# aleflabo/PREGO

Measured on AMD Instinct MI355X. Metric: frames/sec (per-frame action logits) on Assembly101-O TSN features, higher is better.
Workload: dtype fp16; 1 GPU; BASELINE configs[1]: Assembly101-O-test-split-shaped eval set, MiniROAD eval path (rgb+flow fp32 [T,2048] each -> per-frame probs[86] + argmax); clips_per_gpu=182, frames_per_gpu=2306143, min_T=3342, max_T=33981, flow=non-zero (full K=4096 layer1 GEMM), parallelism=clip-sharded dp1, no collective: every rank its own eval-set-sized clip list, weights=random init, seed 20

## Files before the change

### prego_amd/csrc/head_softmax.hip

```cpp
#include "common.h"
#include "kernels.h"
#include <cstdlib>

#define HM 4
template <typename WT, int NTC>
__global__ __launch_bounds__(256) void head_softmax_kernel(
    const WT* __restrict__ Hrelu,
    const WT* __restrict__ Wc,
    const float* __restrict__ bc,
    SlotPlan plan, int row0, int nrows, int HID, int C, int apply_softmax,
    float* const* __restrict__ out_ptrs,
    int* const* __restrict__ argmax_ptrs) {
  constexpr bool BF = (sizeof(WT) == 2);
  const int lane = threadIdx.x & 63, wave = threadIdx.x >> 6;
  const int l15 = lane & 15, l4 = lane >> 4;
  const int rbase = (blockIdx.x * 4 + wave) * 16 * HM;
  if (rbase >= nrows) return;
  int arow[HM];
#pragma unroll
  for (int m = 0; m < HM; ++m) { arow[m] = rbase + m * 16 + l15; if (arow[m] > nrows - 1) arow[m] = nrows - 1; }

  __shared__ unsigned long long s_out[4][64], s_arg[4][64];
  {
    typedef const __attribute__((address_space(4))) int* cint_p;
    cint_p ro_c = (cint_p)plan.rowoff;
    int lo = 0, hi = plan.s_max;
    const int first = __builtin_amdgcn_readfirstlane(row0 + rbase);
    while (hi - lo > 1) {
      const int mid = (lo + hi) >> 1;
      if (ro_c[mid] <= first) lo = mid; else hi = mid;
    }
    int myrow = rbase + lane; if (myrow > nrows - 1) myrow = nrows - 1;
    myrow += row0;
    int a = lo, b = lo + 64 < plan.s_max ? lo + 64 : plan.s_max;
    if (plan.rowoff[b] <= myrow) { a = b; b = plan.s_max; }
    while (b - a > 1) {
      const int mid = (a + b) >> 1;
      if (plan.rowoff[mid] <= myrow) a = mid; else b = mid;
    }
    const int slot = myrow - plan.rowoff[a];
    int k = plan.seg_off[slot];
    const int kend = plan.seg_off[slot + 1];
    while (k + 1 < kend && plan.seg_start[k + 1] <= a) ++k;
    const int clip = plan.seg_clip[k], t = a - plan.seg_start[k];
    float* op = out_ptrs ? out_ptrs[clip] : nullptr;
    int* ap = argmax_ptrs ? argmax_ptrs[clip] : nullptr;
    s_out[wave][lane] = op ? (unsigned long long)(op + (size_t)t * C) : 0ull;
    s_arg[wave][lane] = ap ? (unsigned long long)(ap + t) : 0ull;
  }

  f32x4 acc[HM][NTC];
#pragma unroll
  for (int m = 0; m < HM; ++m)
#pragma unroll
    for (int j = 0; j < NTC; ++j) acc[m][j] = (f32x4){0.f, 0.f, 0.f, 0.f};

  if constexpr (BF) {
    const bf16_t* bp = (const bf16_t*)Wc + (size_t)l15 * HID + 8 * l4;
    for (int k = 0; k < HID; k += 32) {
      bf16x8 af[HM];
#pragma unroll
      for (int m = 0; m < HM; ++m) af[m] = *(const bf16x8*)((const bf16_t*)Hrelu + (size_t)arow[m] * HID + 8 * l4 + k);
#pragma unroll
      for (int j = 0; j < NTC; ++j) {
        const bf16x8 bfr = *(const bf16x8*)(bp + (size_t)j * 16 * HID + k);
#pragma unroll
        for (int m = 0; m < HM; ++m) acc[m][j] = op16<WT>::mfma(af[m], bfr, acc[m][j]);
      }
    }
  } else {
    const float* bp = (const float*)Wc + (size_t)l15 * HID + 4 * l4;
    for (int k = 0; k < HID; k += 16) {
      float4 af[HM];
#pragma unroll
      for (int m = 0; m < HM; ++m) af[m] = *(const float4*)((const float*)Hrelu + (size_t)arow[m] * HID + 4 * l4 + k);
#pragma unroll
      for (int j = 0; j < NTC; ++j) {
        const float4 bv = *(const float4*)(bp + (size_t)j * 16 * HID + k);
#pragma unroll
        for (int m = 0; m < HM; ++m) {
          acc[m][j] = __builtin_amdgcn_mfma_f32_16x16x4f32(af[m].x, bv.x, acc[m][j], 0, 0, 0);
          acc[m][j] = __builtin_amdgcn_mfma_f32_16x16x4f32(af[m].y, bv.y, acc[m][j], 0, 0, 0);
          acc[m][j] = __builtin_amdgcn_mfma_f32_16x16x4f32(af[m].z, bv.z, acc[m][j], 0, 0, 0);
          acc[m][j] = __builtin_amdgcn_mfma_f32_16x16x4f32(af[m].w, bv.w, acc[m][j], 0, 0, 0);
        }
      }
    }
  }

#pragma unroll
  for (int m = 0; m < HM; ++m)
#pragma unroll
  for (int e = 0; e < 4; ++e) {
    float v[NTC];
    float mx = -INFINITY;
    int mi = 0x7fffffff;
#pragma unroll
    for (int j = 0; j < NTC; ++j) {
      const int c = j * 16 + l15;
      v[j] = acc[m][j][e] + bc[c];
      if (c < C && v[j] > mx) { mx = v[j]; mi = c; }
    }
#pragma unroll
    for (int o = 1; o < 16; o <<= 1) {
      const float omx = __shfl_xor(mx, o, 64);
      const int omi = __shfl_xor(mi, o, 64);
      if (omx > mx || (omx == mx && omi < mi)) { mx = omx; mi = omi; }
    }
    float s = 0.f;
    if (apply_softmax) {
#pragma unroll
      for (int j = 0; j < NTC; ++j) {
        const int c = j * 16 + l15;
        v[j] = (c < C) ? __expf(v[j] - mx) : 0.f;
        s += v[j];
      }
#pragma unroll
      for (int o = 1; o < 16; o <<= 1) s += __shfl_xor(s, o, 64);
      const float inv = 1.0f / s;
#pragma unroll
      for (int j = 0; j < NTC; ++j) v[j] *= inv;
    }
    const int rr = m * 16 + l4 * 4 + e;
    if (rbase + rr < nrows) {
      float* op = (float*)s_out[wave][rr];
      if (op) {
#pragma unroll
        for (int j = 0; j < NTC; ++j) {
          const int c = j * 16 + l15;
          if (c < C) op[c] = v[j];
        }
      }
      if (l15 == 0) {
        int* aptr = (int*)s_arg[wave][rr];
        if (aptr) *aptr = mi;
      }
    }
  }
}

template <int NTC, typename OT = bf16_t>
__global__ __launch_bounds__(256, 1) void head_softmax_v2_kernel(
    const bf16_t* __restrict__ Hrelu, const bf16_t* __restrict__ Wc, const float* __restrict__ bc, SlotPlan plan, int row0,
    int nrows, int C, int apply_softmax, float* const* __restrict__ out_ptrs, int* const* __restrict__ argmax_ptrs,
    const int2* __restrict__ rowmap ) {
  constexpr int HID = 1024, KS = 8;
  extern __shared__ __attribute__((aligned(16))) char smem[];
  f32x4* part = (f32x4*)smem;
  constexpr int PSTRIDE = 4 * 2 * NTC * 64;
  const int lane = threadIdx.x & 63, q = __builtin_amdgcn_readfirstlane(threadIdx.x >> 6);
  const int l15 = lane & 15, g = lane >> 4;
  bf16x8 wc[NTC][KS];
#pragma unroll
  for (int j = 0; j < NTC; ++j)
#pragma unroll
    for (int ks = 0; ks < KS; ++ks) wc[j][ks] = *(const bf16x8*)(Wc + (size_t)(j * 16 + l15) * HID + q * 256 + ks * 32 + 8 * g);
  float bias[NTC][4];
#pragma unroll
  for (int j = 0; j < NTC; ++j)
#pragma unroll
    for (int e = 0; e < 4; ++e) bias[j][e] = bc[j * 16 + 4 * g + e];

  const int nblk = (nrows + 31) / 32;
  const int* __restrict__ p_rowoff = plan.rowoff; const int* __restrict__ p_seg_off = plan.seg_off;
  const int* __restrict__ p_seg_clip = plan.seg_clip; const int* __restrict__ p_seg_start = plan.seg_start;
  const int* __restrict__ p_blk = plan.blk_step;
  const int s_max = plan.s_max;
  bf16x8 cur[2][KS], nxt[2][KS];
#define HEAD_LOAD(DST, BLK)                                                                                             \
  do {                                                                                                                  \
    _Pragma("unroll") for (int t = 0; t < 2; ++t) {                                                                     \
      int r_ = (BLK) * 32 + t * 16 + l15; if (r_ > nrows - 1) r_ = nrows - 1;                                           \
      _Pragma("unroll") for (int ks = 0; ks < KS; ++ks) {                                                               \
        const u32x4 v_ = __builtin_nontemporal_load((const u32x4*)(Hrelu + (size_t)r_ * HID + q * 256 + ks * 32 + 8 * g)); \
        DST[t][ks] = __builtin_bit_cast(bf16x8, v_);                                                                    \
      }                                                                                                                 \
    }                                                                                                                   \
  } while (0)
  const int rq = (q & 1) * 16 + l15;
  auto map_row = [&](int b) { int r = b * 32 + rq; return r < nrows ? r : nrows - 1; };
  int blk = blockIdx.x;
  int2 ct = make_int2(0, 0), ctn = make_int2(0, 0);
  if (blk < nblk) {
    if (rowmap != nullptr) ct = rowmap[map_row(blk)];
    HEAD_LOAD(cur, blk);
  }
  int parity = 0;
  for (; blk < nblk; blk += gridDim.x) {
    const int bn = blk + gridDim.x;
    const int bnc = bn < nblk ? bn : blk;
    float* op_raw = nullptr; int* ap_raw = nullptr;
    if (rowmap != nullptr) {
      op_raw = out_ptrs ? out_ptrs[ct.x] : nullptr;
      ap_raw = argmax_ptrs ? argmax_ptrs[ct.x] : nullptr;
      ctn = rowmap[map_row(bnc)];
    }
    __builtin_amdgcn_sched_barrier(0);
    HEAD_LOAD(nxt, bnc);
    __builtin_amdgcn_sched_barrier(0);
    float* op = nullptr; int* ap = nullptr;
    const int myrow = blk * 32 + q * 16 + l15;
    if (q < 2 && myrow < nrows && rowmap == nullptr) {
      const int row = row0 + myrow;
      int lo = p_blk[row >> 5];
      while (lo + 1 < s_max && p_rowoff[lo + 1] <= row) ++lo;
      const int slot = row - p_rowoff[lo];
      int k = p_seg_off[slot];
      const int kend = p_seg_off[slot + 1];
      while (k + 1 < kend && p_seg_start[k + 1] <= lo) ++k;
      const int clip = p_seg_clip[k], t = lo - p_seg_start[k];
      op = out_ptrs ? out_ptrs[clip] : nullptr;
      if (op) op += (size_t)t * C;
      ap = argmax_ptrs ? argmax_ptrs[clip] : nullptr;
      if (ap) ap += t;
    }
    f32x4 acc[2][NTC];
#pragma unroll
    for (int t = 0; t < 2; ++t)
#pragma unroll
      for (int j = 0; j < NTC; ++j) acc[t][j] = (f32x4){0.f, 0.f, 0.f, 0.f};
#pragma unroll
    for (int ks = 0; ks < KS; ++ks)
#pragma unroll
      for (int t = 0; t < 2; ++t)
#pragma unroll
        for (int j = 0; j < NTC; ++j) acc[t][j] = op16<OT>::mfma(wc[j][ks], cur[t][ks], acc[t][j]);
    f32x4* pw = part + parity * PSTRIDE;
    if (q != 0) {
#pragma unroll
      for (int j = 0; j < NTC; ++j) pw[((q * 2 + 0) * NTC + j) * 64 + lane] = acc[0][j];
    }
    if (q != 1) {
#pragma unroll
      for (int j = 0; j < NTC; ++j) pw[((q * 2 + 1) * NTC + j) * 64 + lane] = acc[1][j];
    }
    __syncthreads();
    if (q < 2 && myrow < nrows && rowmap != nullptr) {
      op = op_raw;
      if (op) op += (size_t)ct.y * C;
      ap = ap_raw;
      if (ap) ap += ct.y;
    }
    if (q < 2) {
      float v[NTC][4];
#pragma unroll
      for (int j = 0; j < NTC; ++j) {
        const f32x4 mine = q == 0 ? acc[0][j] : acc[1][j];
        f32x4 sum = (f32x4){0.f, 0.f, 0.f, 0.f};
#pragma unroll
        for (int src = 0; src < 4; ++src) {
          const f32x4 p = (src == q) ? mine : pw[((src * 2 + q) * NTC + j) * 64 + lane];
          sum[0] += p[0]; sum[1] += p[1]; sum[2] += p[2]; sum[3] += p[3];
        }
        v[j][0] = sum[0] + bias[j][0]; v[j][1] = sum[1] + bias[j][1]; v[j][2] = sum[2] + bias[j][2]; v[j][3] = sum[3] + bias[j][3];
      }
      float mx = -INFINITY; int mi = 0x7fffffff;
#pragma unroll
      for (int j = 0; j < NTC; ++j)
#pragma unroll
        for (int e = 0; e < 4; ++e) {
          const int c = j * 16 + 4 * g + e;
          if (c < C && v[j][e] > mx) { mx = v[j][e]; mi = c; }
        }
#pragma unroll
      for (int o = 16; o < 64; o <<= 1) {
        const float omx = __shfl_xor(mx, o, 64);
        const int omi = __shfl_xor(mi, o, 64);
        if (omx > mx || (omx == mx && omi < mi)) { mx = omx; mi = omi; }
      }
      if (apply_softmax) {
        float sm = 0.f;
#pragma unroll
        for (int j = 0; j < NTC; ++j)
#pragma unroll
          for (int e = 0; e < 4; ++e) {
            const int c = j * 16 + 4 * g + e;
            v[j][e] = c < C ? __expf(v[j][e] - mx) : 0.f;
            sm += v[j][e];
          }
        sm += __shfl_xor(sm, 16, 64);
        sm += __shfl_xor(sm, 32, 64);
        const float inv = 1.0f / sm;
#pragma unroll
        for (int j = 0; j < NTC; ++j)
#pragma unroll
          for (int e = 0; e < 4; ++e) v[j][e] *= inv;
      }
      if (op) {
#pragma unroll
        for (int j = 0; j < NTC; ++j) {
          const int c = j * 16 + 4 * g;
          if (c + 3 < C && ((C & 3) == 0)) *(float4*)(op + c) = make_float4(v[j][0], v[j][1], v[j][2], v[j][3]);
          else {
#pragma unroll
            for (int e = 0; e < 4; ++e) if (c + e < C) op[c + e] = v[j][e];
          }
        }
      }
      if (ap && g == 0) *ap = mi;
    }
    parity ^= 1;
    __builtin_amdgcn_sched_barrier(0);
#pragma unroll
    for (int t = 0; t < 2; ++t)
#pragma unroll
      for (int ks = 0; ks < KS; ++ks) cur[t][ks] = nxt[t][ks];
    ct = ctn;
  }
#undef HEAD_LOAD
}

int launch_head_softmax(bool bf16, const void* Hrelu, const void* Wc, const float* bc, const SlotPlan& plan,
                        int row0, int nrows, int hid, int C, int apply_softmax,
                        float* const* out_ptrs, int* const* argmax_ptrs, hipStream_t s, const void* rowmap, bool f16) {
  if (nrows <= 0) return 0;
  const int ntc = (C + 15) / 16;
  static const bool no_v2 = prego_tune_env("PREGO_HEAD_V1") != nullptr;
  if (bf16 && hid == 1024 && ntc <= 6 && !no_v2) {
    const int nblk = (nrows + 31) / 32;
    const int grid2 = nblk < 256 ? nblk : 256;
#define HV2(N)                                                                                                      \
  case N: {                                                                                                         \
    const size_t lds = (size_t)2 * 4 * 2 * N * 64 * 16;                                                             \
    static DeviceOnce once;                                                                                         \
    once.run([&] { (void)hipFuncSetAttribute((const void*)head_softmax_v2_kernel<N>, hipFuncAttributeMaxDynamicSharedMemorySize, (int)lds);   \
                   (void)hipFuncSetAttribute((const void*)head_softmax_v2_kernel<N, f16_t>, hipFuncAttributeMaxDynamicSharedMemorySize, (int)lds); }); \
    if (f16) head_softmax_v2_kernel<N, f16_t><<<grid2, 256, lds, s>>>((const bf16_t*)Hrelu, (const bf16_t*)Wc, bc, plan, row0, nrows, C,  \
                                                                     apply_softmax, out_ptrs, argmax_ptrs, (const int2*)rowmap);    \
    else head_softmax_v2_kernel<N><<<grid2, 256, lds, s>>>((const bf16_t*)Hrelu, (const bf16_t*)Wc, bc, plan, row0, nrows, C,  \
                                                      apply_softmax, out_ptrs, argmax_ptrs, (const int2*)rowmap);    \
    return 0;                                                                                                       \
  }
    switch (ntc) { HV2(1) HV2(2) HV2(3) HV2(4) HV2(5) HV2(6) default: break; }
#undef HV2
  }
  const int grid = (nrows + 64 * HM - 1) / (64 * HM);
#define HL(WT, N)                                                                                             \
  head_softmax_kernel<WT, N><<<grid, 256, 0, s>>>((const WT*)Hrelu, (const WT*)Wc, bc, plan, row0, nrows,     \
                                                  hid, C, apply_softmax, out_ptrs, argmax_ptrs)
#define HD(N)                          \
  case N:                              \
    if (bf16 && f16) HL(f16_t, N);     \
    else if (bf16) HL(bf16_t, N);      \
    else HL(float, N);                 \
    break
  switch (ntc) {
    HD(1); HD(2); HD(3); HD(4); HD(5); HD(6); HD(7); HD(8);
    default: return -1;
  }
#undef HD
#undef HL
  return 0;
}
```

Baseline: 24.29 million frames/s.

## Restructure head softmax kernel into multi-set buffered pipeline with batched row lookup

Rewrites the persistent v2 head kernel to keep two (or three) sets of hidden rows in flight using buffer loads with hardware bounds clamping, refilling each set right after its MFMAs are issued. Destination pointer lookups are batched for 16 iterations into a double-buffered LDS table instead of being computed per iteration. Bias moves to LDS, some weight fragments are pinned to AGPRs, and output stores gain 8-byte-aligned vector paths. This aims to hide global load latency and cut per-iteration scalar and pointer-chasing overhead, in exchange for more registers and LDS and heavier reliance on compiler scheduling hints.

Result: no change. 24.28 million frames/s (-0.1%).

```diff
diff --git a/prego_amd/csrc/head_softmax.hip b/prego_amd/csrc/head_softmax.hip
--- a/prego_amd/csrc/head_softmax.hip
+++ b/prego_amd/csrc/head_softmax.hip
@@ -1,6 +1,7 @@
 #include "common.h"
 #include "kernels.h"
 #include <cstdlib>
+#include <type_traits>
 
 #define HM 4
 template <typename WT, int NTC>
@@ -139,6 +140,10 @@
   }
 }
 
+#ifndef HEAD_DEPTH
+#define HEAD_DEPTH 2
+#endif
+static_assert(HEAD_DEPTH == 2 || HEAD_DEPTH == 3, "the rounds of head_softmax_v2_kernel are written out for two or three sets");
 template <int NTC, typename OT = bf16_t>
 __global__ __launch_bounds__(256, 1) void head_softmax_v2_kernel(
     const bf16_t* __restrict__ Hrelu, const bf16_t* __restrict__ Wc, const float* __restrict__ bc, SlotPlan plan, int row0,
@@ -155,159 +160,211 @@
   for (int j = 0; j < NTC; ++j)
 #pragma unroll
     for (int ks = 0; ks < KS; ++ks) wc[j][ks] = *(const bf16x8*)(Wc + (size_t)(j * 16 + l15) * HID + q * 256 + ks * 32 + 8 * g);
-  float bias[NTC][4];
 #pragma unroll
   for (int j = 0; j < NTC; ++j)
 #pragma unroll
-    for (int e = 0; e < 4; ++e) bias[j][e] = bc[j * 16 + 4 * g + e];
+    for (int ks = 0; ks < KS; ++ks)
+      if ((j * KS + ks) % 3 == 2) asm volatile("" : "+a"(wc[j][ks]));
+  float* sbias = (float*)(part + 2 * PSTRIDE);
+  if (threadIdx.x < NTC * 16) sbias[threadIdx.x] = bc[threadIdx.x];
 
   const int nblk = (nrows + 31) / 32;
   const int* __restrict__ p_rowoff = plan.rowoff; const int* __restrict__ p_seg_off = plan.seg_off;
   const int* __restrict__ p_seg_clip = plan.seg_clip; const int* __restrict__ p_seg_start = plan.seg_start;
   const int* __restrict__ p_blk = plan.blk_step;
   const int s_max = plan.s_max;
-  bf16x8 cur[2][KS], nxt[2][KS];
-#define HEAD_LOAD(DST, BLK)                                                                                             \
-  do {                                                                                                                  \
-    _Pragma("unroll") for (int t = 0; t < 2; ++t) {                                                                     \
-      int r_ = (BLK) * 32 + t * 16 + l15; if (r_ > nrows - 1) r_ = nrows - 1;                                           \
-      _Pragma("unroll") for (int ks = 0; ks < KS; ++ks) {                                                               \
-        const u32x4 v_ = __builtin_nontemporal_load((const u32x4*)(Hrelu + (size_t)r_ * HID + q * 256 + ks * 32 + 8 * g)); \
-        DST[t][ks] = __builtin_bit_cast(bf16x8, v_);                                                                    \
-      }                                                                                                                 \
-    }                                                                                                                   \
-  } while (0)
-  const int rq = (q & 1) * 16 + l15;
-  auto map_row = [&](int b) { int r = b * 32 + rq; return r < nrows ? r : nrows - 1; };
+  constexpr int D = HEAD_DEPTH;
+  const int G = gridDim.x;
+  bf16x8 rows[D][2][KS];
+  const int voff = ((lane & 15) * HID + q * 256 + 8 * g) * 2;
+  auto load_rows = [&](bf16x8 (&dst)[2][KS], int b_) {
+    const int b = __builtin_amdgcn_readfirstlane(b_);
+    const int left = nrows - b * 32;
+    const int nbytes = __builtin_amdgcn_readfirstlane((left < 0 ? 0 : left > 32 ? 32 : left) * HID * 2);
+    const __amdgpu_buffer_rsrc_t rs = __builtin_amdgcn_make_buffer_rsrc((void*)(Hrelu + (size_t)b * 32 * HID), 0, nbytes, 0x00020000);
+    int vo = voff;
+    asm volatile("" : "+v"(vo));
+#pragma unroll
+    for (int t = 0; t < 2; ++t)
+#pragma unroll
+      for (int ks = 0; ks < KS; ++ks)
+        dst[t][ks] = __builtin_bit_cast(bf16x8, __builtin_amdgcn_raw_buffer_load_b128(rs, vo + (t * 16 * HID + ks * 32) * 2, 0, AUX_NT));
+  };
+  constexpr int LOOK = 16;
+  static_assert(LOOK % D == 0, "a look-up sits in front of the refill of set 0");
+  typedef unsigned long long u64;
+  u64* dest = (u64*)(sbias + NTC * 16);
+  auto look_up = [&](int b0, u64* tab) {
+    int tid = threadIdx.x;
+    asm volatile("" : "+v"(tid));
+#pragma unroll
+    for (int e = 0; e < LOOK / 8; ++e) {
+      const int k = e * 8 + (tid >> 5), f = tid & 31;
+      const int myrow = (b0 + k * G) * 32 + f;
+      float* op = nullptr; int* ap = nullptr;
+      if (myrow < nrows) {
+        int clip, t;
+        if (rowmap != nullptr) {
+          const int2 ct = rowmap[myrow];
+          clip = ct.x; t = ct.y;
+        } else {
+          const int row = row0 + myrow;
+          int lo = p_blk[row >> 5];
+          while (lo + 1 < s_max && p_rowoff[lo + 1] <= row) ++lo;
+          const int slot = row - p_rowoff[lo];
+          int kk = p_seg_off[slot];
+          const int kend = p_seg_off[slot + 1];
+          while (kk + 1 < kend && p_seg_start[kk + 1] <= lo) ++kk;
+          clip = p_seg_clip[kk]; t = lo - p_seg_start[kk];
+        }
+        op = out_ptrs ? out_ptrs[clip] : nullptr;
+        if (op) op += (size_t)t * C;
+        ap = argmax_ptrs ? argmax_ptrs[clip] : nullptr;
+        if (ap) ap += t;
+      }
+      tab[(k * 32 + f) * 2 + 0] = (u64)op;
+      tab[(k * 32 + f) * 2 + 1] = (u64)ap;
+    }
+  };
   int blk = blockIdx.x;
-  int2 ct = make_int2(0, 0), ctn = make_int2(0, 0);
-  if (blk < nblk) {
-    if (rowmap != nullptr) ct = rowmap[map_row(blk)];
-    HEAD_LOAD(cur, blk);
-  }
-  int parity = 0;
-  for (; blk < nblk; blk += gridDim.x) {
-    const int bn = blk + gridDim.x;
-    const int bnc = bn < nblk ? bn : blk;
-    float* op_raw = nullptr; int* ap_raw = nullptr;
-    if (rowmap != nullptr) {
-      op_raw = out_ptrs ? out_ptrs[ct.x] : nullptr;
-      ap_raw = argmax_ptrs ? argmax_ptrs[ct.x] : nullptr;
-      ctn = rowmap[map_row(bnc)];
-    }
-    __builtin_amdgcn_sched_barrier(0);
-    HEAD_LOAD(nxt, bnc);
-    __builtin_amdgcn_sched_barrier(0);
-    float* op = nullptr; int* ap = nullptr;
-    const int myrow = blk * 32 + q * 16 + l15;
-    if (q < 2 && myrow < nrows && rowmap == nullptr) {
-      const int row = row0 + myrow;
-      int lo = p_blk[row >> 5];
-      while (lo + 1 < s_max && p_rowoff[lo + 1] <= row) ++lo;
-      const int slot = row - p_rowoff[lo];
-      int k = p_seg_off[slot];
-      const int kend = p_seg_off[slot + 1];
-      while (k + 1 < kend && p_seg_start[k + 1] <= lo) ++k;
-      const int clip = p_seg_clip[k], t = lo - p_seg_start[k];
-      op = out_ptrs ? out_ptrs[clip] : nullptr;
-      if (op) op += (size_t)t * C;
-      ap = argmax_ptrs ? argmax_ptrs[clip] : nullptr;
-      if (ap) ap += t;
-    }
-    f32x4 acc[2][NTC];
-#pragma unroll
-    for (int t = 0; t < 2; ++t)
-#pragma unroll
-      for (int j = 0; j < NTC; ++j) acc[t][j] = (f32x4){0.f, 0.f, 0.f, 0.f};
-#pragma unroll
-    for (int ks = 0; ks < KS; ++ks)
+  if (blk >= nblk) return;
+#pragma unroll
+  for (int s = 0; s < D; ++s) { load_rows(rows[s], blk + s * G); __builtin_amdgcn_sched_barrier(0); }
+#define PIN8(T) "a"(rows[0][T][0]), "a"(rows[0][T][1]), "a"(rows[0][T][2]), "a"(rows[0][T][3]), "a"(rows[0][T][4]), "a"(rows[0][T][5]), "a"(rows[0][T][6]), "a"(rows[0][T][7])
+  static_assert(KS == 8, "PIN8");
+  asm volatile("" : : PIN8(0), PIN8(1));
+#undef PIN8
+  __builtin_amdgcn_sched_barrier(0);
+  int parity = 0, it = 0;
+  auto step = [&](auto set_index) {
+      constexpr int s = decltype(set_index)::value;
+      int lane_ = threadIdx.x & 63;
+      asm volatile("" : "+v"(lane_));
+      const int lane = lane_, l15 = lane & 15, g = lane >> 4;
+      u64* const tab = dest + ((it / LOOK) & 1) * (LOOK * 32 * 2);
+      if (s == 0 && (it & (LOOK - 1)) == 0) look_up(blk, tab);
+      __builtin_amdgcn_sched_barrier(0);
+      f32x4 acc[2][NTC];
 #pragma unroll
       for (int t = 0; t < 2; ++t)
 #pragma unroll
-        for (int j = 0; j < NTC; ++j) acc[t][j] = op16<OT>::mfma(wc[j][ks], cur[t][ks], acc[t][j]);
-    f32x4* pw = part + parity * PSTRIDE;
-    if (q != 0) {
-#pragma unroll
-      for (int j = 0; j < NTC; ++j) pw[((q * 2 + 0) * NTC + j) * 64 + lane] = acc[0][j];
-    }
-    if (q != 1) {
-#pragma unroll
-      for (int j = 0; j < NTC; ++j) pw[((q * 2 + 1) * NTC + j) * 64 + lane] = acc[1][j];
-    }
-    __syncthreads();
-    if (q < 2 && myrow < nrows && rowmap != nullptr) {
-      op = op_raw;
-      if (op) op += (size_t)ct.y * C;
-      ap = ap_raw;
-      if (ap) ap += ct.y;
-    }
-    if (q < 2) {
+        for (int j = 0; j < NTC; ++j) acc[t][j] = (f32x4){0.f, 0.f, 0.f, 0.f};
+#pragma unroll
+      for (int ks = 0; ks < KS; ++ks)
+#pragma unroll
+        for (int t = 0; t < 2; ++t)
+#pragma unroll
+          for (int j = 0; j < NTC; ++j) acc[t][j] = op16<OT>::mfma(wc[j][ks], rows[s][t][ks], acc[t][j]);
+      __builtin_amdgcn_sched_barrier(0);
+      load_rows(rows[s], blk + D * G);
+      __builtin_amdgcn_sched_barrier(0);
+      f32x4* pw = part + parity * PSTRIDE;
+      if (q != 0) {
+#pragma unroll
+        for (int j = 0; j < NTC; ++j) pw[((q * 2 + 0) * NTC + j) * 64 + lane] = acc[0][j];
+      }
+      if (q != 1) {
+#pragma unroll
+        for (int j = 0; j < NTC; ++j) pw[((q * 2 + 1) * NTC + j) * 64 + lane] = acc[1][j];
+      }
+      __syncthreads();
+      typedef __attribute__((address_space(1))) float gfloat;
+      typedef __attribute__((address_space(1))) int gint;
+      typedef __attribute__((address_space(1))) f32x4 gfloat4;
+      typedef __attribute__((ext_vector_type(2))) float f32x2;
+      typedef __attribute__((address_space(1), aligned(8))) f32x4 gfloat4_a8;
+      typedef __attribute__((address_space(1))) f32x2 gfloat2;
+      gfloat* op = nullptr; gint* ap = nullptr;
+      if (q < 2 && blk * 32 + q * 16 + l15 < nrows) {
+        const u64* d = tab + ((it & (LOOK - 1)) * 32 + q * 16 + l15) * 2;
+        op = (gfloat*)d[0];
+        ap = (gint*)d[1];
+      }
       float v[NTC][4];
-#pragma unroll
-      for (int j = 0; j < NTC; ++j) {
-        const f32x4 mine = q == 0 ? acc[0][j] : acc[1][j];
-        f32x4 sum = (f32x4){0.f, 0.f, 0.f, 0.f};
-#pragma unroll
-        for (int src = 0; src < 4; ++src) {
-          const f32x4 p = (src == q) ? mine : pw[((src * 2 + q) * NTC + j) * 64 + lane];
-          sum[0] += p[0]; sum[1] += p[1]; sum[2] += p[2]; sum[3] += p[3];
-        }
-        v[j][0] = sum[0] + bias[j][0]; v[j][1] = sum[1] + bias[j][1]; v[j][2] = sum[2] + bias[j][2]; v[j][3] = sum[3] + bias[j][3];
-      }
-      float mx = -INFINITY; int mi = 0x7fffffff;
-#pragma unroll
-      for (int j = 0; j < NTC; ++j)
-#pragma unroll
-        for (int e = 0; e < 4; ++e) {
-          const int c = j * 16 + 4 * g + e;
-          if (c < C && v[j][e] > mx) { mx = v[j][e]; mi = c; }
-        }
-#pragma unroll
-      for (int o = 16; o < 64; o <<= 1) {
-        const float omx = __shfl_xor(mx, o, 64);
-        const int omi = __shfl_xor(mi, o, 64);
-        if (omx > mx || (omx == mx && omi < mi)) { mx = omx; mi = omi; }
-      }
-      if (apply_softmax) {
-        float sm = 0.f;
+      int mi = 0x7fffffff;
+      if (q < 2) {
+#pragma unroll
+        for (int j = 0; j < NTC; ++j) {
+          const f32x4 mine = q == 0 ? acc[0][j] : acc[1][j];
+          f32x4 sum = (f32x4){0.f, 0.f, 0.f, 0.f};
+#pragma unroll
+          for (int src = 0; src < 4; ++src) {
+            const f32x4 p = (src == q) ? mine : pw[((src * 2 + q) * NTC + j) * 64 + lane];
+            sum[0] += p[0]; sum[1] += p[1]; sum[2] += p[2]; sum[3] += p[3];
+          }
+          const f32x4 bias = *(const f32x4*)(sbias + j * 16 + 4 * g);
+          v[j][0] = sum[0] + bias[0]; v[j][1] = sum[1] + bias[1]; v[j][2] = sum[2] + bias[2]; v[j][3] = sum[3] + bias[3];
+          if (j & 1) __builtin_amdgcn_sched_barrier(0);
+        }
+        float mx = -INFINITY;
 #pragma unroll
         for (int j = 0; j < NTC; ++j)
 #pragma unroll
           for (int e = 0; e < 4; ++e) {
             const int c = j * 16 + 4 * g + e;
-            v[j][e] = c < C ? __expf(v[j][e] - mx) : 0.f;
-            sm += v[j][e];
+            if (c < C && v[j][e] > mx) { mx = v[j][e]; mi = c; }
           }
-        sm += __shfl_xor(sm, 16, 64);
-        sm += __shfl_xor(sm, 32, 64);
-        const float inv = 1.0f / sm;
-#pragma unroll
-        for (int j = 0; j < NTC; ++j)
-#pragma unroll
-          for (int e = 0; e < 4; ++e) v[j][e] *= inv;
-      }
-      if (op) {
-#pragma unroll
-        for (int j = 0; j < NTC; ++j) {
-          const int c = j * 16 + 4 * g;
-          if (c + 3 < C && ((C & 3) == 0)) *(float4*)(op + c) = make_float4(v[j][0], v[j][1], v[j][2], v[j][3]);
-          else {
-#pragma unroll
-            for (int e = 0; e < 4; ++e) if (c + e < C) op[c + e] = v[j][e];
+#pragma unroll
+        for (int o = 16; o < 64; o <<= 1) {
+          const float omx = __shfl_xor(mx, o, 64);
+          const int omi = __shfl_xor(mi, o, 64);
+          if (omx > mx || (omx == mx && omi < mi)) { mx = omx; mi = omi; }
+        }
+        if (apply_softmax) {
+          float sm = 0.f;
+#pragma unroll
+          for (int j = 0; j < NTC; ++j)
+#pragma unroll
+            for (int e = 0; e < 4; ++e) {
+              const int c = j * 16 + 4 * g + e;
+              v[j][e] = c < C ? __expf(v[j][e] - mx) : 0.f;
+              sm += v[j][e];
+            }
+          sm += __shfl_xor(sm, 16, 64);
+          sm += __shfl_xor(sm, 32, 64);
+          const float inv = 1.0f / sm;
+#pragma unroll
+          for (int j = 0; j < NTC; ++j)
+#pragma unroll
+            for (int e = 0; e < 4; ++e) v[j][e] *= inv;
+        }
+      }
+#pragma unroll
+      for (int t = 0; t < 2; ++t)
+#pragma unroll
+        for (int ks = 0; ks < KS; ++ks) asm volatile("" : : "a"(rows[(s + 1) % D][t][ks]));
+      __builtin_amdgcn_sched_barrier(0);
+      if (q < 2) {
+        if (op) {
+          const bool al8 = ((C & 1) == 0) && (((u64)op & 7) == 0);
+#pragma unroll
+          for (int j = 0; j < NTC; ++j) {
+            const int c = j * 16 + 4 * g;
+            if (c + 3 < C && ((C & 3) == 0)) *(gfloat4*)(op + c) = (f32x4){v[j][0], v[j][1], v[j][2], v[j][3]};
+            else if (al8) {
+              if (c + 3 < C) *(gfloat4_a8*)(op + c) = (f32x4){v[j][0], v[j][1], v[j][2], v[j][3]};
+              else if (c + 1 < C) *(gfloat2*)(op + c) = (f32x2){v[j][0], v[j][1]};
+            } else {
+#pragma unroll
+              for (int e = 0; e < 4; ++e) if (c + e < C) op[c + e] = v[j][e];
+            }
           }
         }
-      }
-      if (ap && g == 0) *ap = mi;
-    }
-    parity ^= 1;
-    __builtin_amdgcn_sched_barrier(0);
-#pragma unroll
-    for (int t = 0; t < 2; ++t)
-#pragma unroll
-      for (int ks = 0; ks < KS; ++ks) cur[t][ks] = nxt[t][ks];
-    ct = ctn;
-  }
-#undef HEAD_LOAD
+        if (ap && g == 0) *ap = mi;
+      }
+      parity ^= 1;
+      ++it;
+      blk += G;
+  };
+  while (blk + (D - 1) * G < nblk) {
+    step(std::integral_constant<int, 0>{});
+    step(std::integral_constant<int, 1>{});
+    if constexpr (D > 2) step(std::integral_constant<int, 2>{});
+  }
+  if (blk < nblk) step(std::integral_constant<int, 0>{});
+  if constexpr (D > 2) {
+    if (blk < nblk) step(std::integral_constant<int, 1>{});
+  }
 }
 
 int launch_head_softmax(bool bf16, const void* Hrelu, const void* Wc, const float* bc, const SlotPlan& plan,
@@ -321,7 +378,7 @@
     const int grid2 = nblk < 256 ? nblk : 256;
 #define HV2(N)                                                                                                      \
   case N: {                                                                                                         \
-    const size_t lds = (size_t)2 * 4 * 2 * N * 64 * 16;                                                             \
+    const size_t lds = (size_t)2 * 4 * 2 * N * 64 * 16 + N * 16 * 4 + 2 * 16 * 32 * 16;    \
     static DeviceOnce once;                                                                                         \
     once.run([&] { (void)hipFuncSetAttribute((const void*)head_softmax_v2_kernel<N>, hipFuncAttributeMaxDynamicSharedMemorySize, (int)lds);   \
                    (void)hipFuncSetAttribute((const void*)head_softmax_v2_kernel<N, f16_t>, hipFuncAttributeMaxDynamicSharedMemorySize, (int)lds); }); \
```
